# huakunyang/SummerTTS

Measured on AMD Instinct MI355X. Metric: audio samples/sec (acoustic model + vocoder, phoneme ids -> int16 PCM on host), single_speaker_fast-shaped synthetic blob, higher is better.
Workload: dtype f32 (decoder trunk convs AND the reverse flow's WaveNet convs (wn_flow.hip, one-utterance calls): fp32 operands as 2 fp16 terms = 22-23 of their 24 mantissa bits, 3 fp16 MFMA products per fp32 product, f32 accumulation -- measured error in `parity`, same tolerance as the exact-fp32 leg; batches addi

## Files before the change

summertts_amd/csrc/wn_flow.hip:

```cpp
#include "conv_bf3_dev.hpp"

namespace sts {

#ifdef STS_TILE_TRACE
int tile_trace_bind_flow(long long* buf, unsigned capacity_records) { return tile_trace_bind(buf, capacity_records); }
#endif

constexpr int FL_WIN = 64;
constexpr int FL_NT = 32;
constexpr int FL_UR = 2;
constexpr int FL_MAXG = 8;

__device__ __forceinline__ unsigned fl_b_off(int chunk, int pos, int half, int plane, int plane_bytes) {
    return (unsigned)(chunk * 2 * plane_bytes + plane * plane_bytes + pos * 32 + ((half ^ ((pos >> 3) & 1)) << 4));
}

__device__ __forceinline__ void split4h(const float (&x)[4], unsigned (&hi)[2], unsigned (&lo)[2], float& amax) {
#pragma unroll
    for (int d = 0; d < 2; d++) {
        const f32x2 v = {x[2 * d], x[2 * d + 1]};
        const f16x2 h = __builtin_convertvector(v, f16x2);
#if STS_SPLIT_MIX
        const f32x2 v2 = v * 2048.f;
        const unsigned hu = __builtin_bit_cast(unsigned, h);
        unsigned l = 0u;
        asm("v_fma_mixlo_f16 %0, %1, %2, %3 op_sel:[0,0,0] op_sel_hi:[1,0,0]\n\t"
            "v_fma_mixhi_f16 %0, %1, %2, %4 op_sel:[1,0,0] op_sel_hi:[1,0,0]"
            : "+v"(l) : "v"(hu), "s"(-2048.0f), "v"(v2[0]), "v"(v2[1]));
        hi[d] = hu;
        lo[d] = l;
#else
        const f32x2 r = (v - __builtin_convertvector(h, f32x2)) * 2048.f;
        const f16x2 l = __builtin_convertvector(r, f16x2);
        hi[d] = __builtin_bit_cast(unsigned, h);
        lo[d] = __builtin_bit_cast(unsigned, l);
#endif
        amax = __builtin_fmaxf(amax, __builtin_fmaxf(__builtin_fabsf(v[0]), __builtin_fabsf(v[1])));
    }
}

constexpr int FL_WAVES = 8;
constexpr int FL_GSTEPS = 16;
template <bool L0>
__global__ __launch_bounds__(64 * FL_WAVES) __attribute__((amdgpu_waves_per_eu(2, 2))) void flow_layer_kernel(FlowLayerArgs a) {
    extern __shared__ __attribute__((aligned(16))) unsigned char fsm[];
    const int Gp = (a.G + 7) & ~7;
    const int g = (int)(blockIdx.x % (unsigned)Gp);
    if (g >= a.G) return;
    const int rest = (int)(blockIdx.x / (unsigned)Gp);
    const int ntile = (a.max_len + FL_NT - 1) / FL_NT;
    const int b = rest / ntile, tile = rest - b * ntile;
    const int len = uni(seg_len(a.seg, b));
    const int n0 = tile * FL_NT;
    if (n0 >= len) return;
    const size_t base = (size_t)uni(seg_start(a.seg, b));
    const int tid = threadIdx.x, lane = tid & 63, wave = __builtin_amdgcn_readfirstlane(tid >> 6);
    const int l31 = lane & 31, half = lane >> 5;
    const int H = a.H, hc = a.half, Cg = a.Cg, halo = a.halo;
    const int W = FL_NT + 2 * halo;
    const int NCH = H >> 4;
    const int PLANE = FL_WIN * 32;
    unsigned char* const R_h = fsm;
    unsigned char* const R_x = fsm + (size_t)NCH * 2 * PLANE;
    unsigned char* const R_a = R_x + (size_t)FL_WAVES * 4096;
    const int APL = FL_NT * 32;
    float amax = 0.f;
    constexpr int RG = 2, KS = FL_WAVES / RG;
    const int rt_l = wave % RG, kq = wave / RG;
#ifdef STS_TILE_TRACE
    long long* tt_rec = tt_open(3 + (L0 ? 1 : 0), g);
    TT_STAMP(0);
#endif

    const int nrtg = (2 * H) >> 5;
    const int c_lo = NCH * kq / KS, c_hi = NCH * (kq + 1) / KS;
    const int nsteps = (c_hi - c_lo) * a.k;
    u32x4 fa[FL_GSTEPS][1][2];
    auto gate_prefetch = [&](auto lo_c, auto hi_c) {
        constexpr int lo = decltype(lo_c)::value, hi = decltype(hi_c)::value;
        const rsrc_t wrs = make_rsrc(a.w_gate, (unsigned)((size_t)NCH * a.k * nrtg * 2048u));
        const int rt = g * RG + rt_l;
#pragma unroll
        for (int s = lo; s < hi; s++) {
            const int c = c_lo + s / a.k, j = s - (s / a.k) * a.k;
            const unsigned o = s < nsteps ? (unsigned)(((c * a.k + j) * nrtg + rt) * 2048 + lane * 16) : kOOB;
#pragma unroll
            for (int pl = 0; pl < 2; pl++) fa[s][0][pl] = __builtin_bit_cast(u32x4, __builtin_amdgcn_raw_buffer_load_b128(wrs, (int)o, pl * 1024, 0));
        }
    };
    using I0 = std::integral_constant<int, 0>; using IH = std::integral_constant<int, FL_GSTEPS / 2>; using IE = std::integral_constant<int, FL_GSTEPS>;
    const int ntc = a.rows_c >> 5;
    const int nkc = Cg >> 4;
    u32x4 fc[2][2][1][2];
    auto c_prefetch = [&]() {
        const rsrc_t wrs = make_rsrc(a.w_c, (unsigned)((size_t)NCH * ntc * 2048u));
#pragma unroll
        for (int ti = 0; ti < 2; ti++) {
            const int t = wave + FL_WAVES * ti;
#pragma unroll
            for (int cs = 0; cs < 2; cs++)
#pragma unroll
                for (int pl = 0; pl < 2; pl++) {
                    const unsigned off = t < ntc && cs < nkc ? (unsigned)(((g * nkc + cs) * ntc + t) * 2048 + pl * 1024 + lane * 16) : kOOB;
                    fc[ti][cs][0][pl] = __builtin_bit_cast(u32x4, __builtin_amdgcn_raw_buffer_load_b128(wrs, (int)off, 0, 0));
                }
        }
    };

    f32x4u mold[2][4];
    auto m_prefetch = [&]() {
        const rsrc_t rm = make_rsrc(a.macc + (size_t)g * a.macc_stride, a.macc_init ? 0u : (unsigned)(((size_t)a.tot * hc) * 4u));
#pragma unroll
        for (int ti = 0; ti < 2; ti++) {
            const int t = wave + FL_WAVES * ti;
#pragma unroll
            for (int q = 0; q < 4; q++) {
                const int c = t * 32 + 8 * q + 4 * half - a.rows_res;
                const bool okm = t < ntc && c >= 0 && c + 3 < hc && n0 + l31 < len;
                const unsigned off = okm ? (unsigned)(((base + (size_t)(n0 + l31)) * hc + c) * 4u) : kOOB;
                mold[ti][q] = __builtin_bit_cast(f32x4u, __builtin_amdgcn_raw_buffer_load_b128(rm, (int)off, 0, 0));
            }
        }
    };

    if constexpr (!L0) {
        gate_prefetch(I0{}, IH{});
        const int qpp = H >> 2;
        const int nunit = W * qpp;
        const unsigned span = (unsigned)(((size_t)a.tot * H) * 4u);
        const rsrc_t rh = make_rsrc(a.h_in, span);
        for (int u0 = 0; u0 < nunit; u0 += 64 * FL_WAVES * FL_UR) {
            f32x4u v[FL_UR], p[FL_UR][FL_MAXG];
            int pw[FL_UR], q4[FL_UR]; bool ok[FL_UR];
#pragma unroll
            for (int r = 0; r < FL_UR; r++) {
                const int u = u0 + r * 64 * FL_WAVES + tid;
                pw[r] = u / qpp; q4[r] = u - pw[r] * qpp;
                const int pos = n0 - halo + pw[r];
                ok[r] = u < nunit && pos >= 0 && pos < len;
                const unsigned off = ok[r] ? (unsigned)(((base + (size_t)pos) * H + (size_t)q4[r] * 4) * 4u) : kOOB;
                v[r] = __builtin_bit_cast(f32x4u, __builtin_amdgcn_raw_buffer_load_b128(rh, (int)off, 0, 0));
#pragma unroll
                for (int s = 0; s < FL_MAXG; s++) {
                    const rsrc_t rp = make_rsrc(a.part_in + (size_t)s * a.part_stride, s < a.part_n ? span : 0u);
                    p[r][s] = __builtin_bit_cast(f32x4u, __builtin_amdgcn_raw_buffer_load_b128(rp, (int)off, 0, 0));
                }
            }
#pragma unroll
            for (int r = 0; r < FL_UR; r++) {
                const int u = u0 + r * 64 * FL_WAVES + tid;
                if (u >= nunit) continue;
                f32x4u s4 = v[r];
#pragma unroll
                for (int s = 0; s < FL_MAXG; s++) s4 += p[r][s];
                const int ch = q4[r] * 4;
                if (ok[r] && pw[r] >= halo && pw[r] < halo + FL_NT && ch >= g * Cg && ch < (g + 1) * Cg)
                    *(f32x4u*)(a.h_out + (base + (size_t)(n0 - halo + pw[r])) * H + ch) = s4;
                const float x4[4] = {s4[0], s4[1], s4[2], s4[3]};
                unsigned hi[2], lo[2];
                split4h(x4, hi, lo, amax);
                const int chunk = ch >> 4, hf = (ch >> 3) & 1, qd = (ch >> 2) & 1;
                unsigned char* d = R_h + fl_b_off(chunk, pw[r], hf, 0, PLANE) + qd * 8;
                *(uint2*)d = uint2{hi[0], hi[1]};
                *(uint2*)(d + PLANE) = uint2{lo[0], lo[1]};
            }
        }
        TT_STAMP(1);
        gate_prefetch(IH{}, IE{});
        c_prefetch();
        m_prefetch();
    } else {
        gate_prefetch(I0{}, IH{});
        const int nrt = H >> 5, nk = hc >> 4;
        u32x4 fp[8][1][2];
        {
            const rsrc_t wrs = make_rsrc(a.w_pre, (unsigned)((size_t)nk * nrt * 2048u));
#pragma unroll
            for (int cs = 0; cs < 8; cs++)
#pragma unroll
                for (int pl = 0; pl < 2; pl++) {
                    const unsigned o = wave < nrt && cs < nk ? (unsigned)((cs * nrt + wave) * 2048 + pl * 1024 + lane * 16) : kOOB;
                    fp[cs][0][pl] = __builtin_bit_cast(u32x4, __builtin_amdgcn_raw_buffer_load_b128(wrs, (int)o, 0, 0));
                }
        }
        const int qpp = hc >> 2;
        const int nunit = W * qpp;
        const unsigned pspan = (unsigned)(((size_t)a.tot * hc) * 4u);
        for (int u0 = 0; u0 < nunit; u0 += 64 * FL_WAVES * FL_UR) {
            float zv[FL_UR][4]; f32x4u p[FL_UR][FL_MAXG];
            int pw[FL_UR], q4[FL_UR]; bool ok[FL_UR];
#pragma unroll
            for (int r = 0; r < FL_UR; r++) {
                const int u = u0 + r * 64 * FL_WAVES + tid;
                q4[r] = u / W; pw[r] = u - q4[r] * W;
                const int pos = n0 - halo + pw[r];
                ok[r] = u < nunit && pos >= 0 && pos < len;
                const size_t zo = (size_t)(q4[r] * 4) * a.x0_ld + base + (size_t)(ok[r] ? pos : 0);
#pragma unroll
                for (int e = 0; e < 4; e++) zv[r][e] = ok[r] ? a.x0[zo + (size_t)e * a.x0_ld] : 0.f;
                const unsigned off = ok[r] ? (unsigned)(((base + (size_t)pos) * hc + (size_t)q4[r] * 4) * 4u) : kOOB;
#pragma unroll
                for (int s = 0; s < FL_MAXG; s++) {
                    const rsrc_t rp = make_rsrc(a.pend + (size_t)s * a.pend_stride, s < a.pend_n ? pspan : 0u);
                    p[r][s] = __builtin_bit_cast(f32x4u, __builtin_amdgcn_raw_buffer_load_b128(rp, (int)off, 0, 0));
                }
            }
#pragma unroll
            for (int r = 0; r < FL_UR; r++) {
                const int u = u0 + r * 64 * FL_WAVES + tid;
                if (u >= nunit) continue;
                f32x4u s4 = {zv[r][0], zv[r][1], zv[r][2], zv[r][3]};
#pragma unroll
                for (int s = 0; s < FL_MAXG; s++) s4 += p[r][s];
                const int ch = q4[r] * 4;
                if (a.x0_out && ok[r] && pw[r] >= halo && pw[r] < halo + FL_NT && (q4[r] % a.G) == g) {
                    float* zp = a.x0_out + (size_t)ch * a.x0_out_ld + base + (size_t)(n0 - halo + pw[r]);
#pragma unroll
                    for (int e = 0; e < 4; e++) zp[(size_t)e * a.x0_out_ld] = s4[e];
                }
                const float x4[4] = {s4[0], s4[1], s4[2], s4[3]};
                unsigned hi[2], lo[2];
                split4h(x4, hi, lo, amax);
                const int chunk = ch >> 4, hf = (ch >> 3) & 1, qd = (ch >> 2) & 1;
                unsigned char* d = R_x + fl_b_off(chunk, pw[r], hf, 0, PLANE) + qd * 8;
                *(uint2*)d = uint2{hi[0], hi[1]};
                *(uint2*)(d + PLANE) = uint2{lo[0], lo[1]};
            }
        }
        __syncthreads();
        TT_STAMP(1);
        gate_prefetch(IH{}, IE{});
        if (wave < nrt) {
            const int rt = wave;
            f32x16 acc[1][2];
#pragma unroll
            for (int ct = 0; ct < 2; ct++)
#pragma unroll
                for (int r = 0; r < 16; r++) acc[0][ct][r] = 0.f;
#pragma unroll
            for (int cs = 0; cs < 8; cs++)
                if (cs < nk) {
                    u32x4 fb[2][2];
#pragma unroll
                    for (int ct = 0; ct < 2; ct++)
#pragma unroll
                        for (int pl = 0; pl < 2; pl++) fb[ct][pl] = *(const u32x4*)(R_x + fl_b_off(cs, ct * 32 + l31, half, pl, PLANE));
                    step_mfmas<1, 1, 2, 2, 2>(acc, fp[cs], fb);
                }
#pragma unroll
            for (int ct = 0; ct < 2; ct++) {
                const int pw_ = ct * 32 + l31;
                const int pos = n0 - halo + pw_;
                const bool inside = pos >= 0 && pos < len && pw_ < W;
#pragma unroll
                for (int hh = 0; hh < 2; hh++) {
                    float v8[8];
#pragma unroll
                    for (int e = 0; e < 8; e++) {
                        const int row = rt * 32 + hh * 16 + 8 * (e >> 2) + 4 * half + (e & 3);
                        const float t1 = acc[0][ct][hh * 8 + e] * a.s_pre + (a.b_pre ? a.b_pre[row] : 0.f);
                        v8[e] = inside ? t1 : 0.f;
                    }
                    u32x4 ph, pl;
                    split8h(v8, ph, pl, amax);
                    unsigned char* d = R_h + fl_b_off(rt * 2 + hh, pw_, half, 0, PLANE);
                    *(u32x4*)d = ph;
                    *(u32x4*)(d + PLANE) = pl;
                    if (inside && pw_ >= halo && pw_ < halo + FL_NT) {
#pragma unroll
                        for (int qd = 0; qd < 2; qd++) {
                            const int ch = rt * 32 + hh * 16 + 8 * qd + 4 * half;
                            if (ch >= g * Cg && ch < (g + 1) * Cg)
                                *(f32x4u*)(a.h_out + (base + (size_t)pos) * H + ch) = f32x4u{v8[4 * qd], v8[4 * qd + 1], v8[4 * qd + 2], v8[4 * qd + 3]};
                        }
                    }
                }
            }
        }
        c_prefetch();
        m_prefetch();
    }
    __syncthreads();
    TT_STAMP(2);

    f32x16 acc[1][1], acc1[1][1];
#pragma unroll
    for (int r = 0; r < 16; r++) { acc[0][0][r] = 0.f; acc1[0][0][r] = 0.f; }
    {
        u32x4 fb[2][1][2];
        auto load_b = [&](int s, u32x4 (&dst)[1][2]) {
            const int ss = s < nsteps ? s : 0;
            const int c = c_lo + ss / a.k, j = ss - (ss / a.k) * a.k;
#pragma unroll
            for (int pl = 0; pl < 2; pl++) dst[0][pl] = *(const u32x4*)(R_h + fl_b_off(c, l31 + j, half, pl, PLANE));
        };
        load_b(0, fb[0]);
        static_for<0, FL_GSTEPS>([&](auto sc) {
            constexpr int s = decltype(sc)::value;
            if (s < nsteps) {
                load_b(s + 1, fb[(s + 1) % 2]);
                if constexpr (s % 2 == 0) step_mfmas<1, 1, 1, 2, 2>(acc, fa[s], fb[s % 2]);
                else step_mfmas<1, 1, 1, 2, 2>(acc1, fa[s], fb[s % 2]);
            }
        });
#pragma unroll
        for (int r = 0; r < 16; r++) acc[0][0][r] += acc1[0][0][r];
    }
    TT_STAMP(3);
    float* const red = (float*)R_x;
    __syncthreads();
#pragma unroll
    for (int r = 0; r < 16; r++) red[((size_t)(kq * RG + rt_l) * 16 + r) * 64 + lane] = acc[0][0][r];
    __syncthreads();
    {
        const int rowb = (g * RG + rt_l) * 32;
        float gv[2];
#pragma unroll
        for (int i = 0; i < 2; i++) {
            const int r = 2 * kq + i;
            float t = 0.f, sg = 0.f;
            for (int q = 0; q < KS; q++) {
                t += red[((size_t)(q * RG + rt_l) * 16 + r) * 64 + lane];
                sg += red[((size_t)(q * RG + rt_l) * 16 + r + 8) * 64 + lane];
            }
            const int rowp = rowb + (r & 3) + 8 * (r >> 2) + 4 * half;
            t = t * a.s_gate + (a.b_gate ? a.b_gate[rowp] : 0.f);
            sg = sg * a.s_gate + (a.b_gate ? a.b_gate[rowp + 16] : 0.f);
            if (a.ubias) { t += a.ubias[(size_t)rowp * a.ubias_ld + b]; sg += a.ubias[(size_t)(rowp + 16) * a.ubias_ld + b]; }
            gv[i] = tanh_ref(t) * sigmoid_ref(sg);
        }
        const f32x2 v = {gv[0], gv[1]};
        const f16x2 hh = __builtin_convertvector(v, f16x2);
        const f32x2 rr = (v - __builtin_convertvector(hh, f32x2)) * 2048.f;
        const f16x2 ll = __builtin_convertvector(rr, f16x2);
        amax = __builtin_fmaxf(amax, __builtin_fmaxf(__builtin_fabsf(v[0]), __builtin_fabsf(v[1])));
        unsigned char* d = R_a + (size_t)rt_l * 2 * APL + l31 * 32 + ((half ^ ((l31 >> 3) & 1)) << 4) + kq * 4;
        *(unsigned*)d = __builtin_bit_cast(unsigned, hh);
        *(unsigned*)(d + APL) = __builtin_bit_cast(unsigned, ll);
    }
    __syncthreads();
    TT_STAMP(4);

    const int pos_o = n0 + l31;
    const bool col_ok = pos_o < len;
#pragma unroll
    for (int ti = 0; ti < 2; ti++) {
        const int t = wave + FL_WAVES * ti;
        if (t >= ntc) continue;
        f32x16 ac[1][1];
#pragma unroll
        for (int r = 0; r < 16; r++) ac[0][0][r] = 0.f;
#pragma unroll
        for (int cs = 0; cs < 2; cs++)
            if (cs < nkc) {
                u32x4 fb[1][2];
                const unsigned char* sp = R_a + (size_t)cs * 2 * APL + l31 * 32 + ((half ^ ((l31 >> 3) & 1)) << 4);
                fb[0][0] = *(const u32x4*)sp;
                fb[0][1] = *(const u32x4*)(sp + APL);
                step_mfmas<1, 1, 1, 2, 2>(ac, fc[ti][cs], fb);
            }
        if (!col_ok) continue;
        const int row0 = t * 32;
#pragma unroll
        for (int q = 0; q < 4; q++) {
            const int row = row0 + 8 * q + 4 * half;
            f32x4u v = {ac[0][0][4 * q] * a.s_c, ac[0][0][4 * q + 1] * a.s_c, ac[0][0][4 * q + 2] * a.s_c, ac[0][0][4 * q + 3] * a.s_c};
            if (row < a.rows_res) {
                if (g == 0 && a.b_res) v += *(const f32x4u*)(a.b_res + row);
                if (row + 3 < H) *(f32x4u*)(a.part_out + (size_t)g * a.part_stride + (base + (size_t)pos_o) * H + row) = v;
            } else {
                const int c = row - a.rows_res;
                if (c + 3 < hc) {
                    float* mp = a.macc + (size_t)g * a.macc_stride + (base + (size_t)pos_o) * hc + c;
                    if (a.macc_init) { if (g == 0 && a.b_m) v += *(const f32x4u*)(a.b_m + c); }
                    else v += mold[ti][q];
                    *(f32x4u*)mp = v;
                }
            }
        }
    }
    if (amax > kH2Limit && a.ovf) *a.ovf = 1u;
#ifdef STS_TILE_TRACE
    asm volatile("s_waitcnt vmcnt(0)" ::: "memory");
    TT_STAMP(5);
    TT_CLOSE();
#endif
}

__global__ __launch_bounds__(256) void flow_finish_kernel(FlowFinishArgs a) {
    const int b = blockIdx.y;
    const int len = seg_len(a.seg, b);
    const size_t base = (size_t)seg_start(a.seg, b);
    const int idx = blockIdx.x * 256 + threadIdx.x;
    const int qpp = a.half >> 2;
    const int q = idx / a.max_len, pos = idx - q * a.max_len;
    if (q >= qpp || pos >= len) return;
    f32x4u s4;
#pragma unroll
    for (int e = 0; e < 4; e++) s4[e] = a.src[(size_t)(q * 4 + e) * a.src_ld + base + pos];
    for (int s = 0; s < a.n; s++) s4 += *(const f32x4u*)(a.macc + (size_t)s * a.macc_stride + (base + (size_t)pos) * a.half + q * 4);
#pragma unroll
    for (int e = 0; e < 4; e++) a.dst[(size_t)(q * 4 + e) * a.dst_ld + base + pos] = s4[e];
}

bool flow_layer_shape_ok(int H, int half, int k, int dil, int n_layers) {
    if (H < 32 || H % 32 != 0 || H > 256 || half < 16 || half % 16 != 0 || half % 4 != 0 || half > 128) return false;
    if (!(k & 1) || k < 1 || dil != 1 || (k - 1) > FL_WIN - FL_NT || n_layers < 1) return false;
    const int Cg = 32, G = H / Cg;
    if (G > FL_MAXG) return false;
    const int RG = 2, KS = FL_WAVES / RG, NCH = H / 16;
    if (((NCH + KS - 1) / KS) * k > FL_GSTEPS) return false;
    if (half / 16 > 8 || H / 32 > FL_WAVES) return false;
    const int rows_c = ((H + half) + 31) / 32 * 32;
    return rows_c / 32 <= 2 * FL_WAVES;
}
int flow_layer_groups(int H) { return H / 32; }

static size_t flow_lds_bytes(int H) {
    const size_t h = (size_t)(H / 16) * 2 * FL_WIN * 32;
    return h + (size_t)FL_WAVES * 4096 + (size_t)4 * 2 * FL_NT * 32 + 256;
}

void flow_layer(const FlowLayerArgs& a, hipStream_t st) {
    if (a.max_len <= 0 || a.B <= 0) return;
    const int Gp = (a.G + 7) & ~7;
    const int ntile = (a.max_len + FL_NT - 1) / FL_NT;
    const size_t lds = flow_lds_bytes(a.H);
    if (a.layer == 0) {
        (void)hipFuncSetAttribute((const void*)flow_layer_kernel<true>, hipFuncAttributeMaxDynamicSharedMemorySize, (int)lds);
        hipLaunchKernelGGL(flow_layer_kernel<true>, dim3((unsigned)((size_t)ntile * a.B * Gp)), dim3(64 * FL_WAVES), lds, st, a);
    } else {
        (void)hipFuncSetAttribute((const void*)flow_layer_kernel<false>, hipFuncAttributeMaxDynamicSharedMemorySize, (int)lds);
        hipLaunchKernelGGL(flow_layer_kernel<false>, dim3((unsigned)((size_t)ntile * a.B * Gp)), dim3(64 * FL_WAVES), lds, st, a);
    }
}

void flow_finish(const FlowFinishArgs& a, hipStream_t st) {
    if (a.max_len <= 0 || a.B <= 0) return;
    const long n = (long)(a.half >> 2) * a.max_len;
    hipLaunchKernelGGL(flow_finish_kernel, dim3((unsigned)((n + 255) / 256), a.B), dim3(256), 0, st, a);
}

}
```

Measured before the change: 67.28 million.

## Stage flow-layer biases in LDS and remap grid to drop padded group blocks

Each block now loads all bias vectors (pre, gate, res, m, and the per-utterance conditioning bias) into registers once at kernel start, then writes them to a new LDS region. The epilogues read biases from LDS instead of issuing scattered global loads, notably the strided ubias reads. The grid mapping also changes: the group index is no longer padded to 8, which removes blocks that exited immediately, and 8 consecutive blocks now cover 8 tiles of the same group so they share weights in cache. This costs extra LDS and some registers per block, and the padded unit count can still launch a few idle blocks.

```diff
diff --git a/summertts_amd/csrc/wn_flow.hip b/summertts_amd/csrc/wn_flow.hip
--- a/summertts_amd/csrc/wn_flow.hip
+++ b/summertts_amd/csrc/wn_flow.hip
@@ -10,6 +10,7 @@
 constexpr int FL_NT = 32;
 constexpr int FL_UR = 2;
 constexpr int FL_MAXG = 8;
+constexpr int FL_BIAS = 6 * 256 + 128;
 
 __device__ __forceinline__ unsigned fl_b_off(int chunk, int pos, int half, int plane, int plane_bytes) {
     return (unsigned)(chunk * 2 * plane_bytes + plane * plane_bytes + pos * 32 + ((half ^ ((pos >> 3) & 1)) << 4));
@@ -44,11 +45,11 @@
 template <bool L0>
 __global__ __launch_bounds__(64 * FL_WAVES) __attribute__((amdgpu_waves_per_eu(2, 2))) void flow_layer_kernel(FlowLayerArgs a) {
     extern __shared__ __attribute__((aligned(16))) unsigned char fsm[];
-    const int Gp = (a.G + 7) & ~7;
-    const int g = (int)(blockIdx.x % (unsigned)Gp);
-    if (g >= a.G) return;
-    const int rest = (int)(blockIdx.x / (unsigned)Gp);
     const int ntile = (a.max_len + FL_NT - 1) / FL_NT;
+    const int slot = (int)(blockIdx.x >> 3);
+    const int g = slot % a.G;
+    const int rest = (slot / a.G) * 8 + (int)(blockIdx.x & 7u);
+    if (rest >= ntile * a.B) return;
     const int b = rest / ntile, tile = rest - b * ntile;
     const int len = uni(seg_len(a.seg, b));
     const int n0 = tile * FL_NT;
@@ -63,6 +64,7 @@
     unsigned char* const R_h = fsm;
     unsigned char* const R_x = fsm + (size_t)NCH * 2 * PLANE;
     unsigned char* const R_a = R_x + (size_t)FL_WAVES * 4096;
+    float* const R_b = (float*)(R_a + (size_t)4 * 2 * FL_NT * 32);
     const int APL = FL_NT * 32;
     float amax = 0.f;
     constexpr int RG = 2, KS = FL_WAVES / RG;
@@ -71,6 +73,28 @@
     long long* tt_rec = tt_open(3 + (L0 ? 1 : 0), g);
     TT_STAMP(0);
 #endif
+
+    const int nbias = 6 * H + hc;
+    constexpr int FL_BJ = (FL_BIAS + 64 * FL_WAVES - 1) / (64 * FL_WAVES);
+    float bv[FL_BJ];
+#pragma unroll
+    for (int j = 0; j < FL_BJ; j++) {
+        const int i = tid + 64 * FL_WAVES * j;
+        const float* src = nullptr;
+        if (i < H) { if (L0 && a.b_pre) src = a.b_pre + i; }
+        else if (i < 3 * H) { if (a.b_gate) src = a.b_gate + (i - H); }
+        else if (i < 4 * H) { if (a.rows_res > 0 && a.b_res) src = a.b_res + (i - 3 * H); }
+        else if (i < 4 * H + hc) { if (a.macc_init && a.b_m) src = a.b_m + (i - 4 * H); }
+        else if (i < nbias) { if (a.ubias) src = a.ubias + (size_t)(i - 4 * H - hc) * a.ubias_ld + b; }
+        bv[j] = src ? *src : 0.f;
+    }
+    auto bias_stage = [&]() {
+#pragma unroll
+        for (int j = 0; j < FL_BJ; j++) {
+            const int i = tid + 64 * FL_WAVES * j;
+            if (i < nbias) R_b[i] = bv[j];
+        }
+    };
 
     const int nrtg = (2 * H) >> 5;
     const int c_lo = NCH * kq / KS, c_hi = NCH * (kq + 1) / KS;
@@ -165,6 +189,7 @@
                 *(uint2*)(d + PLANE) = uint2{lo[0], lo[1]};
             }
         }
+        bias_stage();
         TT_STAMP(1);
         gate_prefetch(IH{}, IE{});
         c_prefetch();
@@ -227,6 +252,7 @@
                 *(uint2*)(d + PLANE) = uint2{lo[0], lo[1]};
             }
         }
+        bias_stage();
         __syncthreads();
         TT_STAMP(1);
         gate_prefetch(IH{}, IE{});
@@ -258,7 +284,7 @@
 #pragma unroll
                     for (int e = 0; e < 8; e++) {
                         const int row = rt * 32 + hh * 16 + 8 * (e >> 2) + 4 * half + (e & 3);
-                        const float t1 = acc[0][ct][hh * 8 + e] * a.s_pre + (a.b_pre ? a.b_pre[row] : 0.f);
+                        const float t1 = acc[0][ct][hh * 8 + e] * a.s_pre + R_b[row];
                         v8[e] = inside ? t1 : 0.f;
                     }
                     u32x4 ph, pl;
@@ -324,9 +350,9 @@
                 sg += red[((size_t)(q * RG + rt_l) * 16 + r + 8) * 64 + lane];
             }
             const int rowp = rowb + (r & 3) + 8 * (r >> 2) + 4 * half;
-            t = t * a.s_gate + (a.b_gate ? a.b_gate[rowp] : 0.f);
-            sg = sg * a.s_gate + (a.b_gate ? a.b_gate[rowp + 16] : 0.f);
-            if (a.ubias) { t += a.ubias[(size_t)rowp * a.ubias_ld + b]; sg += a.ubias[(size_t)(rowp + 16) * a.ubias_ld + b]; }
+            t = t * a.s_gate + R_b[H + rowp];
+            sg = sg * a.s_gate + R_b[H + rowp + 16];
+            if (a.ubias) { t += R_b[4 * H + hc + rowp]; sg += R_b[4 * H + hc + rowp + 16]; }
             gv[i] = tanh_ref(t) * sigmoid_ref(sg);
         }
         const f32x2 v = {gv[0], gv[1]};
@@ -366,13 +392,13 @@
             const int row = row0 + 8 * q + 4 * half;
             f32x4u v = {ac[0][0][4 * q] * a.s_c, ac[0][0][4 * q + 1] * a.s_c, ac[0][0][4 * q + 2] * a.s_c, ac[0][0][4 * q + 3] * a.s_c};
             if (row < a.rows_res) {
-                if (g == 0 && a.b_res) v += *(const f32x4u*)(a.b_res + row);
+                if (g == 0 && a.b_res) v += *(const f32x4u*)(R_b + 3 * H + row);
                 if (row + 3 < H) *(f32x4u*)(a.part_out + (size_t)g * a.part_stride + (base + (size_t)pos_o) * H + row) = v;
             } else {
                 const int c = row - a.rows_res;
                 if (c + 3 < hc) {
                     float* mp = a.macc + (size_t)g * a.macc_stride + (base + (size_t)pos_o) * hc + c;
-                    if (a.macc_init) { if (g == 0 && a.b_m) v += *(const f32x4u*)(a.b_m + c); }
+                    if (a.macc_init) { if (g == 0 && a.b_m) v += *(const f32x4u*)(R_b + 4 * H + c); }
                     else v += mold[ti][q];
                     *(f32x4u*)mp = v;
                 }
@@ -418,20 +444,24 @@
 
 static size_t flow_lds_bytes(int H) {
     const size_t h = (size_t)(H / 16) * 2 * FL_WIN * 32;
-    return h + (size_t)FL_WAVES * 4096 + (size_t)4 * 2 * FL_NT * 32 + 256;
+    return h + (size_t)FL_WAVES * 4096 + (size_t)4 * 2 * FL_NT * 32 + (size_t)FL_BIAS * 4 + 256;
+}
+
+static unsigned flow_grid(const FlowLayerArgs& a) {
+    const long units = (long)((a.max_len + FL_NT - 1) / FL_NT) * a.B;
+    return (unsigned)((units + 7) / 8 * 8 * a.G);
 }
 
 void flow_layer(const FlowLayerArgs& a, hipStream_t st) {
     if (a.max_len <= 0 || a.B <= 0) return;
-    const int Gp = (a.G + 7) & ~7;
-    const int ntile = (a.max_len + FL_NT - 1) / FL_NT;
+    const unsigned grid = flow_grid(a);
     const size_t lds = flow_lds_bytes(a.H);
     if (a.layer == 0) {
         (void)hipFuncSetAttribute((const void*)flow_layer_kernel<true>, hipFuncAttributeMaxDynamicSharedMemorySize, (int)lds);
-        hipLaunchKernelGGL(flow_layer_kernel<true>, dim3((unsigned)((size_t)ntile * a.B * Gp)), dim3(64 * FL_WAVES), lds, st, a);
+        hipLaunchKernelGGL(flow_layer_kernel<true>, dim3(grid), dim3(64 * FL_WAVES), lds, st, a);
     } else {
         (void)hipFuncSetAttribute((const void*)flow_layer_kernel<false>, hipFuncAttributeMaxDynamicSharedMemorySize, (int)lds);
-        hipLaunchKernelGGL(flow_layer_kernel<false>, dim3((unsigned)((size_t)ntile * a.B * Gp)), dim3(64 * FL_WAVES), lds, st, a);
+        hipLaunchKernelGGL(flow_layer_kernel<false>, dim3(grid), dim3(64 * FL_WAVES), lds, st, a);
     }
 }
 
```

Result: no change. 67.00 million, median of 4 (-0.4%).
